# unknownue/puflow

Measured on AMD Instinct MI355X. Metric: patches/sec x4 2048->8192 (PU1K discrete, eval), higher is better.
Workload: dtype f32 (split-fp16 MFMA products, fp32 accumulate); 1 GPU; BASELINE configs[1]: PU1K discrete x4 inference, 32 x 2048-pt patches per GPU (fp32-parity mode); patches_per_gpu=32, total_batch=32, npoint=2048

## Files before the change

include/puflow_hip.h:

```cpp
#ifndef PUFLOW_HIP_H
#define PUFLOW_HIP_H

#ifdef __cplusplus
extern "C" {
#endif

#define PF_OK 0
#define PF_ERR_NULL (-1)
#define PF_ERR_SHAPE (-2)
#define PF_ERR_UNSUPPORTED (-3)
#define PF_ERR_LAUNCH (-4)
#define PF_ERR_WORKSPACE (-5)

int pf_version(void);
const char* pf_error_string(int code);

int pf_knn(const float* p1, const float* p2, int B, int N, int M, int K, int* idx_out, float* dist_out, void* stream);

int pf_nn1(const float* p1, const float* p2, int B, int N, int M, float* dist_out, int* idx_out, void* stream);

int pf_edgeconv(int cfg, const float* pq_or_xyz, const float* tab, const int* idx, const float* wfrag, float* out,
                int B, int N, void* stream);

int pf_edgeconv_tuned(int cfg, int variant, const float* pq_or_xyz, const float* tab, const int* idx,
                      const float* wfrag, float* out, int B, int N, void* stream);

int pf_edgeconv_pq(int unit, const float* pq_or_xyz, const int* idx, const float* wfrag, float* out, const float* w,
                   const long long* off, float* pq_next, int B, int N, int fuse, void* stream);

int pf_pq_gemm(int unit, const float* h, const float* w, const long long* off, float* pq_next, int T, void* stream);
int pf_cond(int unit, const float* h, const float* w, const long long* off, float* c, float* st, float* cp, int T,
            void* stream);
int pf_post(int unit, const float* h, const float* w, const long long* off, float* c, float* st, float* cp,
            float* pq_next, int T, void* stream);
int pf_test_act_pairn(const float* x, int n, float inv, float slope, unsigned* old_h, unsigned* old_l, unsigned* new_h,
                      unsigned* new_l, void* stream);
int pf_cond_all(const float* const* h, const float* w, const long long* off, float* const* c, float* st, float* cp, int T,
                void* stream);

int pf_flow_fwd(const float* xyz, const float* cp, const float* st, const float* w, float* z, float* ld_pt, int T,
                void* stream);

int pf_flow_inv(const float* u, const float* cp, const float* st, const float* w, float* x, int T, int R, void* stream);

int pf_logp(const float* z, const float* ld_pt, float ld_const, int B, int N, float* ldj, float* lpsum, float* logp,
            void* stream);

long long pf_flow_fwd_logp_ws_floats(int B, int N);
int pf_flow_fwd_logp(const float* xyz, const float* cp, const float* st, const float* w, float* z, float* ld_pt,
                     float ld_const, int B, int N, float* ldj, float* lpsum, float* logp, float* ws, void* stream);

int pf_interp(const float* xyz, const float* z, const int* idx16, const float* w, const long long* off, float* u_out,
              int B, int N, int R, void* stream);

int pf_interp_weights(const float* xyz, const int* idx16, const float* w, const long long* off, float* aw_out, int B, int N,
                      void* stream);
int pf_flow_inv_interp(const float* aw, const float* z, const int* idx16, const float* cp, const float* st, const float* w,
                       float* x, int B, int N, int R, void* stream);

int pf_chamfer_fwd(const float* x, const float* y, int B, int N, int M, float* dist1, int* idx1, float* dist2,
                   int* idx2, float* per_sample, float* mean_sum, void* stream);

int pf_chamfer_bwd(const float* x, const float* y, const int* idx1, const int* idx2, const float* g1, const float* g2,
                   float* gx, float* gy, int B, int N, int M, void* stream);
int pf_chamfer_bwd_det(const float* x, const float* y, const int* idx1, const int* idx2, const float* g1, const float* g2,
                       float* gx, float* gy, int B, int N, int M, void* stream);

int pf_emd_forward(const float* xyz1, const float* xyz2, float* dist, int* assignment, float* price,
                   int* assignment_inv, int* bid, float* bid_increments, float* max_increments, int* unass_idx,
                   int* max_idx, float eps, int iters, int B, int n, void* stream);

int pf_emd_forward_ex(const float* xyz1, const float* xyz2, float* dist, int* assignment, float* price,
                      int* assignment_inv, int* bid, float* bid_increments, float* max_increments, int* unass_idx,
// ... 410 lines not shown
```

puflow_amd/csrc/flow.hip:

```cpp
#include <hip/hip_runtime.h>
#include "pf_api_internal.h"
#include "pf_mfma.h"
#include "pf_wave.h"

#ifndef PF_FLOW_NW
#define PF_FLOW_NW 16
#endif
#ifndef PF_FLOW_NW_FWD
#define PF_FLOW_NW_FWD 16
#endif

namespace {

constexpr int FLOW_REC = 5360;
constexpr float LOG2PI_F = 1.8378770664093453f;

struct FlowArgs {
    const float* in;
    const float* cp;
    const float* st;
    const float* w;
    float* out;
    float* ld_pt;
    int T;
    int R;
    int rows;
    int ntiles;
    float* part;
    unsigned* counter;
    float* ldj; float* lps; float* logp;
    float ld_const;
    int B, N;
    const float* aw;
    const float* z;
    const int* idx;
};

struct FlowCond { f4 cp[4]; f4 s0, s1; };

__device__ __forceinline__ FlowCond flow_cond(const float* __restrict__ cp, const float* __restrict__ st, int T, int u,
                                              int pt, int q) {
    FlowCond c;
    const float* cr = cp + ((size_t)u * T + pt) * 64 + 4 * q;
#pragma unroll
    for (int cb = 0; cb < 4; ++cb) c.cp[cb] = *reinterpret_cast<const f4*>(cr + cb * 16);
    const float* sr = st + ((size_t)u * T + pt) * 8;
    c.s0 = *reinterpret_cast<const f4*>(sr);
    c.s1 = *reinterpret_cast<const f4*>(sr + 4);
    return c;
}

template <int TD>
__device__ __forceinline__ void coupling_net(const float* rec , int lane, int q, const FlowCond& c,
                                             const float (&h1)[2], float (&o)[2]) {
    PfPairN hp[1][2];
    const float i2 = rec[5352], i4 = rec[5353];
    {
        f4 hid[4];
#pragma unroll
        for (int cb = 0; cb < 4; ++cb) {
            const f4 wa = *reinterpret_cast<const f4*>(rec + 5200 + (cb * 16 + 4 * q) * 2);
            const f4 wb = *reinterpret_cast<const f4*>(rec + 5200 + (cb * 16 + 4 * q) * 2 + 4);
            f4 v = c.cp[cb];
            v.x = fmaf(wa.x, h1[0], v.x); v.y = fmaf(wa.z, h1[0], v.y);
            v.z = fmaf(wb.x, h1[0], v.z); v.w = fmaf(wb.z, h1[0], v.w);
// ... 7 lines not shown
        hp[0][1] = pf_act_pairn(hid[2], hid[3], 0.01f);
    }
    const PfW2Lds ws{reinterpret_cast<const u4*>(rec), lane};
    f4 h2[1][4];
#pragma unroll
    for (int ob = 0; ob < 4; ++ob) h2[0][ob] = pf_bias(rec + 5120, ob, q);
    pf_mmn<false, 4, 2, 2>(ws, 0, hp, h2);
    hp[0][0] = pf_act_pairn(h2[0][0], h2[0][1], i2, 0.01f);
    hp[0][1] = pf_act_pairn(h2[0][2], h2[0][3], i2, 0.01f);
    f4 acc[1][1];
    acc[0][0] = *reinterpret_cast<const f4*>(rec + 5184 + 4 * q);
    pf_mmn<false, 1, 2, 2>(ws, 8, hp, acc);
    o[0] = acc[0][0].x * i4; o[1] = acc[0][0].y * i4;
}

template <bool INV, int NW>
__global__ __launch_bounds__(NW * 64) void flow_kernel(FlowArgs a) {
    const int lane = threadIdx.x & 63, wave = threadIdx.x >> 6;
    const int col = lane & 15, q = lane >> 4;
    __shared__ f4 wl[6 * FLOW_REC / 4];
    pf_stage_lds(wl, reinterpret_cast<const f4*>(a.w), 6 * FLOW_REC / 4);
    __syncthreads();
    const float* wlf = reinterpret_cast<const float*>(wl);

    for (int tile = blockIdx.x; tile < a.ntiles; tile += gridDim.x) {
        const int g = (tile * NW + wave) * 16 + col;
        const bool ok = g < a.rows;
        const int row = ok ? g : a.rows - 1;
        const int pt = row / a.R;
        float v[3], ld = 0.f;
        if (INV && a.aw) {
            const int r = row - pt * a.R, bN = (pt / a.N) * a.N;
            const int4 j0 = *reinterpret_cast<const int4*>(a.idx + (size_t)pt * 16), j1 = *reinterpret_cast<const int4*>(a.idx + (size_t)pt * 16 + 4);
            const int jj[8] = {j0.x, j0.y, j0.z, j0.w, j1.x, j1.y, j1.z, j1.w};
            float sk[8][3];
#pragma unroll
            for (int k = 0; k < 8; ++k) {
                const float wk = a.aw[((size_t)pt * 8 + k) * 4 + r];
                const float* zz = a.z + (size_t)(bN + jj[k]) * 3;
#pragma unroll
                for (int c = 0; c < 3; ++c) sk[k][c] = __fmul_rn(wk, zz[c]);
            }
#pragma unroll
            for (int c = 0; c < 3; ++c)
                v[c] = __fadd_rn(__fadd_rn(__fadd_rn(sk[0][c], sk[1][c]), __fadd_rn(sk[2][c], sk[3][c])),
                                 __fadd_rn(__fadd_rn(sk[4][c], sk[5][c]), __fadd_rn(sk[6][c], sk[7][c])));
        } else {
#pragma unroll
            for (int c = 0; c < 3; ++c) v[c] = a.in[(size_t)row * 3 + c];
        }
        FlowCond cn = flow_cond(a.cp, a.st, a.T, INV ? 5 : 0, pt, q);

        pf_static_for<0, 6>([&](auto uc) {
            constexpr int i = decltype(uc)::value;
            constexpr int u = INV ? 5 - i : i;
            constexpr int TD = (u % 2 == 0) ? 1 : 2;
            const float* rec = wlf + u * FLOW_REC;
            const float* fc = rec + 5328;
            const FlowCond c = cn;
            if constexpr (i < 5) cn = flow_cond(a.cp, a.st, a.T, INV ? u - 1 : u + 1, pt, q);
            __builtin_amdgcn_sched_barrier(0);
            const float s[3] = {c.s0.x, c.s0.y, c.s0.z}, t[3] = {c.s0.w, c.s1.x, c.s1.y};
            float h1[2], o[2];
            if constexpr (!INV) {
                const float x0 = v[0], x1 = v[1], x2 = v[2];
#pragma unroll
                for (int k = 0; k < 3; ++k)
                    v[k] = fmaf(fc[3 * k + 2], x2, fmaf(fc[3 * k + 1], x1, fmaf(fc[3 * k], x0, fc[9 + k])));
                h1[0] = v[0]; h1[1] = v[1];
                coupling_net<TD>(rec, lane, q, c, h1, o);
                if (TD == 1) { v[1] -= o[0]; v[2] -= o[1]; } else { v[2] -= o[0]; }
                const float y0 = v[2], y1 = v[1], y2 = v[0];
                v[0] = (y0 - t[0]) * expf(-s[0]);
                v[1] = (y1 - t[1]) * expf(-s[1]);
                v[2] = (y2 - t[2]) * expf(-s[2]);
                ld -= (s[0] + s[1]) + s[2];
            } else {
                const float y0 = fmaf(v[0], expf(s[0]), t[0]);
                const float y1 = fmaf(v[1], expf(s[1]), t[1]);
                const float y2 = fmaf(v[2], expf(s[2]), t[2]);
                v[0] = y2; v[1] = y1; v[2] = y0;
                h1[0] = v[0]; h1[1] = v[1];
                coupling_net<TD>(rec, lane, q, c, h1, o);
                if (TD == 1) { v[1] += o[0]; v[2] += o[1]; } else { v[2] += o[0]; }
                const float x0 = v[0], x1 = v[1], x2 = v[2];
#pragma unroll
                for (int k = 0; k < 3; ++k)
                    v[k] = fmaf(fc[12 + 3 * k + 2], x2, fmaf(fc[12 + 3 * k + 1], x1, fmaf(fc[12 + 3 * k], x0, fc[21 + k])));
            }
        });

        if (ok && q == 0) {
            a.out[(size_t)row * 3 + 0] = v[0];
            a.out[(size_t)row * 3 + 1] = v[1];
            a.out[(size_t)row * 3 + 2] = v[2];
// ... 39 lines not shown
                a.lps[b] = accz + l;
                if (b < NW * 64) sa[b] = accz + l;
            }
        }
        __syncthreads();
        float tot = 0.f;
        if (tid == 0)
            for (int b = 0; b < a.B; ++b) tot += b < NW * 64 ? sa[b] : a.lps[b];
        if (tid == 0) {
            *a.logp = -tot / (float)a.B;
            PF_ST(a.counter, 0u);
        }
    }
}

template <bool INV, int NW>
int launch_nw(FlowArgs a, hipStream_t s) {
    a.ntiles = (a.rows + NW * 16 - 1) / (NW * 16);
    const int grid = a.ntiles < 256 ? a.ntiles : 256;
    hipLaunchKernelGGL((flow_kernel<INV, NW>), dim3(grid), dim3(NW * 64), 0, s, a);
    return pf_last_launch_status();
}

template <bool INV>
int launch(FlowArgs a, hipStream_t s) {
    constexpr int NWMAX = INV ? PF_FLOW_NW : PF_FLOW_NW_FWD;
    const int wt = (a.rows + 15) / 16;
    if (wt >= 200 * NWMAX) return launch_nw<INV, NWMAX>(a, s);
    if (wt >= 200 * 8) return launch_nw<INV, 8>(a, s);
    return launch_nw<INV, 4>(a, s);
}

__global__ __launch_bounds__(256) void logp_batch_kernel(const float* __restrict__ z, const float* __restrict__ ld_pt,
                                                        float ld_const, int N, float* __restrict__ ldj,
                                                        float* __restrict__ lpsum) {
    __shared__ float sa[256], sb[256];
    const int b = blockIdx.x, tid = threadIdx.x;
    float accl = 0.f, accz = 0.f;
    for (int n = tid; n < N; n += 256) {
        accl += ld_pt[(size_t)b * N + n];
        const float* zz = z + ((size_t)b * N + n) * 3;
        accz += -0.5f * (zz[0] * zz[0] + LOG2PI_F) + -0.5f * (zz[1] * zz[1] + LOG2PI_F) + -0.5f * (zz[2] * zz[2] + LOG2PI_F);
    }
    sa[tid] = accl; sb[tid] = accz;
    __syncthreads();
// ... 33 lines not shown
                                float ld_const, int B, int N, float* ldj, float* lpsum, float* logp, float* ws, void* stream) {
    if (!xyz || !cp || !st || !w || !z || !ld_pt || !ldj || !lpsum || !logp || !ws) return PF_ERR_NULL;
    if (B <= 0 || N <= 0 || (long long)B * N > (1ll << 30)) return PF_ERR_SHAPE;
    const int T = B * N;
    if (N % 16 != 0) {
        const int rc = pf_flow_fwd(xyz, cp, st, w, z, ld_pt, T, stream);
        return rc != PF_OK ? rc : pf_logp(z, ld_pt, ld_const, B, N, ldj, lpsum, logp, stream);
    }
    FlowArgs a{};
    a.in = xyz; a.cp = cp; a.st = st; a.w = w; a.out = z; a.ld_pt = ld_pt; a.T = T; a.R = 1; a.rows = T;
    a.part = ws; a.counter = reinterpret_cast<unsigned*>(ws + 2 * (T / 16));
    a.ldj = ldj; a.lps = lpsum; a.logp = logp; a.ld_const = ld_const; a.B = B; a.N = N;
    return launch<false>(a, (hipStream_t)stream);
}

extern "C" int pf_flow_inv(const float* u, const float* cp, const float* st, const float* w, float* x, int T, int R,
                           void* stream) {
    if (!u || !cp || !st || !w || !x) return PF_ERR_NULL;
    if (T <= 0 || R <= 0 || (long long)T * R > (1ll << 30)) return PF_ERR_SHAPE;
    FlowArgs a{};
    a.in = u; a.cp = cp; a.st = st; a.w = w; a.out = x; a.ld_pt = nullptr; a.T = T; a.R = R; a.rows = T * R;
    return launch<true>(a, (hipStream_t)stream);
}

extern "C" int pf_flow_inv_interp(const float* aw, const float* z, const int* idx16, const float* cp, const float* st, const float* w,
                                  float* x, int B, int N, int R, void* stream) {
    if (!aw || !z || !idx16 || !cp || !st || !w || !x) return PF_ERR_NULL;
    if (B <= 0 || N < 8 || (long long)B * N * R > (1ll << 30)) return PF_ERR_SHAPE;
    if (R < 1 || R > 4) return PF_ERR_UNSUPPORTED;
    FlowArgs a{};
    a.in = nullptr; a.cp = cp; a.st = st; a.w = w; a.out = x; a.ld_pt = nullptr; a.T = B * N; a.R = R; a.rows = B * N * R;
    a.aw = aw; a.z = z; a.idx = idx16; a.N = N;
    return launch<true>(a, (hipStream_t)stream);
}

extern "C" int pf_logp(const float* z, const float* ld_pt, float ld_const, int B, int N, float* ldj, float* lpsum,
                       float* logp, void* stream) {
    if (!z || !ld_pt || !ldj || !lpsum || !logp) return PF_ERR_NULL;
    if (B <= 0 || N <= 0) return PF_ERR_SHAPE;
    hipStream_t s = (hipStream_t)stream;
    hipLaunchKernelGGL(logp_batch_kernel, dim3(B), dim3(256), 0, s, z, ld_pt, ld_const, N, ldj, lpsum);
    hipLaunchKernelGGL(logp_final_kernel, dim3(1), dim3(64), 0, s, lpsum, B, logp);
    return pf_last_launch_status();
}
```

puflow_amd/csrc/pointwise.hip:

```cpp
#include <hip/hip_runtime.h>
#include "pf_api_internal.h"
#include "pf_mfma.h"
#include "pf_pq.h"

namespace {

struct PqArgs {
    const float* h;
    const u4* w;
    const float* bias;
    const float* scales;
    float* pq;
    int T, ntiles, NT, nrounds;
    float inv;
};

template <int ODIM, int ROWS, int NW>
__global__ __launch_bounds__(NW * 64) void pq_gemm_kernel(PqArgs a) {
    constexpr int HB = ODIM / 16, CP = (HB + 1) / 2, OBT = ROWS / 16, RB = OBT / NW, NTMAX = 16;
    static_assert(OBT % NW == 0, "rows split evenly over the waves");
    const int lane = threadIdx.x & 63, wave = threadIdx.x >> 6;
    const int col = lane & 15, q = lane >> 4;
    __shared__ u4 bl[NTMAX * PQ_TILE_U4<CP>];
    h8 wh[RB][CP], wl[RB][CP];
// ... 33 lines not shown
    nt = nt < 1 ? 1 : (nt > 16 ? 16 : nt);
    a.NT = nt;
    a.nrounds = (a.ntiles + nt - 1) / nt;
    const int grid = a.nrounds < 256 ? a.nrounds : 256;
    hipLaunchKernelGGL((pq_gemm_kernel<ODIM, ROWS, NW>), dim3(grid), dim3(NW * 64), 0, s, a);
    return pf_last_launch_status();
}

struct CondArgs {
    const float* h;
    const float* w;
    long long off[13];
    float* c;
    float* st;
    float* cp;
    int T, ntiles;
    int contiguous;
};

__device__ __forceinline__ f4 pf_scale(f4 v, float k) { return v * k; }

template <int ODIM>
constexpr int cond_lds_bytes() { return ((ODIM / 32) * ((ODIM / 16 + 1) / 2) + 12 * ((ODIM / 32 + 1) / 2) + 20) * 2048; }

template <int ODIM, int CDIM, int NW>
__device__ __forceinline__ void cond_body(const CondArgs& a, u4* wl, int tile0, int tstride) {
    constexpr int HB = ODIM / 16, MB = ODIM / 32, CB = CDIM / 16;
    constexpr int HP = (HB + 1) / 2, MP = (MB + 1) / 2;
    constexpr int F_M1 = 0, F_H1 = F_M1 + MB * HP, F_S2 = F_H1 + 12 * MP, F_T2 = F_S2 + 8, F_ST4 = F_T2 + 8, F_END = F_ST4 + 4;
    const int lane = threadIdx.x & 63, wave = threadIdx.x >> 6;
    const int col = lane & 15, q = lane >> 4;
    static_assert(F_END * 2048 == cond_lds_bytes<ODIM>(), "LDS size formula");
    {
        auto stage = [&](int f0, int nf, long long off) {
            const u4* src = reinterpret_cast<const u4*>(a.w + off);
// ... 74 lines not shown
            PfPairN h1p[1][2];
            h1p[0][0] = pf_act_pairn(h1[0][0], h1[0][1], iH1, 0.01f);
            h1p[0][1] = pf_act_pairn(h1[0][2], h1[0][3], iH1, 0.01f);
            f4 h2[1][4];
#pragma unroll
            for (int o = 0; o < 4; ++o) h2[0][o] = pf_bias(net == 0 ? bS2 : bT2, o, q);
            if constexpr (net == 0) pf_mmn<false, 4, 2, 2>(wsS2, 0, h1p, h2); else pf_mmn<false, 4, 2, 2>(wsT2, 0, h1p, h2);
            const float i2 = net == 0 ? iS2 : iT2;
            h2p[0][2 * net + 0] = pf_act_pairn(h2[0][0], h2[0][1], i2, 0.01f);
            h2p[0][2 * net + 1] = pf_act_pairn(h2[0][2], h2[0][3], i2, 0.01f);
        });
        {
            f4 acc[1][1];
            acc[0][0] = pf_bias(bST4, 0, q);
            pf_mmn<false, 1, 4, 4>(wsST4, 0, h2p, acc);
            if (ok && q < 2) *reinterpret_cast<f4*>(a.st + (size_t)pt * 8 + 4 * q) = pf_scale(acc[0][0], iST4);
        }
    }
}

#ifndef PF_COND_NW
#define PF_COND_NW 12
#endif
constexpr int COND_NW = PF_COND_NW;

template <int ODIM, int CDIM>
__global__ __launch_bounds__(COND_NW * 64) void cond_kernel(CondArgs a) {
    extern __shared__ u4 cond_lds[];
    cond_body<ODIM, CDIM, COND_NW>(a, cond_lds, blockIdx.x, gridDim.x);
}

// ... 81 lines not shown
                       int T, void* stream) {
    if (!h || !w || !off || !st || !cp) return PF_ERR_NULL;
    if (T <= 0) return PF_ERR_SHAPE;
    CondArgs a{};
    a.h = h; a.w = w; a.c = c; a.st = st; a.cp = cp; a.T = T;
    for (int i = 0; i < 13; ++i) a.off[i] = off[i];
    hipStream_t s = (hipStream_t)stream;
    switch (unit) {
        case 0: return launch_cond<32, 32>(a, s);
        case 1: return launch_cond<64, 64>(a, s);
        case 2: case 3: case 4: case 5: return launch_cond<128, 128>(a, s);
        default: return PF_ERR_UNSUPPORTED;
    }
}

extern "C" int pf_cond_all(const float* const* h, const float* w, const long long* off, float* const* c, float* st, float* cp,
                           int T, void* stream) {
    if (!h || !w || !off || (!st != !cp) || (!st && !c)) return PF_ERR_NULL;
    if (T <= 0) return PF_ERR_SHAPE;
    CondAllArgs g{};
    const int ntiles = (T + 15) / 16;
    const int wgt = (ntiles + COND_NW - 1) / COND_NW;
    static const int share_big[6] = {32, 32, 48, 48, 48, 48}, share_small[6] = {24, 32, 50, 50, 50, 50};
    const int* share = wgt <= 50 ? share_small : share_big;
    g.first[0] = 0;
    for (int u = 0; u < 6; ++u) {
        if (!h[u]) return PF_ERR_NULL;
        CondArgs& a = g.u[u];
        a.h = h[u]; a.w = w; a.c = c ? c[u] : nullptr; a.st = st ? st + (size_t)u * T * 8 : nullptr; a.cp = cp ? cp + (size_t)u * T * 64 : nullptr; a.T = T;
        a.ntiles = ntiles;
        for (int i = 0; i < 13; ++i) a.off[i] = off[u * 13 + i];
        a.contiguous = cond_contiguous(a.off, u == 0 ? 32 : (u == 1 ? 64 : 128));
        const int n = wgt < share[u] ? wgt : share[u];
        g.first[u + 1] = g.first[u] + n;
    }
    constexpr int lds = cond_lds_bytes<128>();
    allow_lds(cond_all_kernel, lds);
    hipLaunchKernelGGL(cond_all_kernel, dim3(g.first[6]), dim3(COND_NW * 64), lds, (hipStream_t)stream, g);
    return pf_last_launch_status();
}

extern "C" int pf_post(int unit, const float* h, const float* w, const long long* off, float* c, float* st, float* cp,
                       float* pq_next, int T, void* stream) {
    if (unit < 5) {
        if (!pq_next) return PF_ERR_NULL;
        const int rc = pf_pq_gemm(unit, h, w, off, pq_next, T, stream);
        if (rc != PF_OK) return rc;
    }
    return pf_cond(unit, h, w, off, c, st, cp, T, stream);
}

namespace {
__global__ void act_pairn_test_kernel(const float* __restrict__ x, int n8, float inv, float slope, u4* __restrict__ old_h,
                                      u4* __restrict__ old_l, u4* __restrict__ new_h, u4* __restrict__ new_l) {
// ... 5 lines not shown
    old_h[i] = __builtin_bit_cast(u4, o.h); old_l[i] = __builtin_bit_cast(u4, o.l);
    new_h[i] = __builtin_bit_cast(u4, n.h); new_l[i] = __builtin_bit_cast(u4, n.l);
}
}

extern "C" int pf_test_act_pairn(const float* x, int n, float inv, float slope, unsigned* old_h, unsigned* old_l,
                                 unsigned* new_h, unsigned* new_l, void* stream) {
    if (!x || !old_h || !old_l || !new_h || !new_l) return PF_ERR_NULL;
    if (n <= 0 || n % 8 != 0) return PF_ERR_SHAPE;
    const int n8 = n / 8;
    hipLaunchKernelGGL(act_pairn_test_kernel, dim3((n8 + 63) / 64), dim3(64), 0, (hipStream_t)stream, x, n8, inv, slope,
                       reinterpret_cast<u4*>(old_h), reinterpret_cast<u4*>(old_l), reinterpret_cast<u4*>(new_h),
                       reinterpret_cast<u4*>(new_l));
    return pf_last_launch_status();
}
```

puflow_amd/interpflow.py:

```python
from __future__ import annotations

import os
from typing import List, Optional, Tuple

import numpy as np
import torch
import torch.nn as nn
from torch import Tensor

from . import _lib
from .packing import COND_CHANNELS, FEAT_CHANNELS, GROWTH, NUM_BLOCKS, fold_state_dict, pack_plan

_EC_CFG = [0, 1, 2, 2, 2, 2]
_CHECK_FINITE = os.environ.get("PF_CHECK_FINITE", "0") == "1"


def _conv_bn(cin: int, cout: int, slope: float) -> nn.Sequential:
    return nn.Sequential(nn.Conv2d(cin, cout, kernel_size=1), nn.BatchNorm2d(cout), nn.LeakyReLU(slope))


class _EdgeConvParams(nn.Module):

    def __init__(self, cin: int, odim: int, growth: int):
        super().__init__()
# ... 60 lines not shown
    def __init__(self):
        super().__init__()
        self.knn_context = _Holder()
        self.knn_context.distance_encoder = _Holder()
        self.knn_context.distance_encoder.mlp = nn.Sequential(
            *_conv_bn(10, 64, 0.01), *_conv_bn(64, 64, 0.01), nn.Conv2d(64, 128, kernel_size=1))
        self.knn_context.feat_conv = _EdgeConvParams(3, 128, 16)
        self.weight_unit = _Holder()
        self.weight_unit.mlp = nn.Sequential(
            *_conv_bn(256, 128, 0.01), *_conv_bn(128, 64, 0.01), nn.Conv2d(64, 32, kernel_size=1))


class CondList(list):
    cp: Tensor
    st: Tensor


def _host_state_dict(sd):
    out, groups = {}, {}
    for k, v in sd.items():
        v = v.detach()
        if v.is_cuda:
            groups.setdefault(v.dtype, []).append((k, v))
        else:
            out[k] = v
    for dt, items in groups.items():
        flat = torch.cat([v.reshape(-1) for _, v in items]).cpu()
        pos = 0
        for k, v in items:
            out[k] = flat[pos:pos + v.numel()].reshape(v.shape)
# ... 68 lines not shown
                w = self.ec1n_w[u] if u < 2 else self.ec4_w[u]
                _lib.check(self.lib.pf_edgeconv_pq(u, src, idx16.data_ptr(), self._p(w), h.data_ptr(), self.base, self.post[u],
                                                   nxt.data_ptr(), B, N, self.fuse_pq, s), f"pf_edgeconv_pq[{u}]")

            def pq_gemm(u=u, h=h, nxt=nxt):
                _lib.check(self.lib.pf_pq_gemm(u, h.data_ptr(), self.base, self.post[u], nxt.data_ptr(), T, s), f"pf_pq_gemm[{u}]")

            if u + 1 == NUM_BLOCKS:
                yield h, [(f"edgeconv{u}", ec)]
            elif fused:
                yield h, [(f"edgeconv{u}+pq", ec_pq)]
            else:
                yield h, [(f"edgeconv{u}", ec), (f"pq{u}", pq_gemm)]

    def features(self, xyz: Tensor, idx16: Tensor, want_cs: bool, cs_only: bool = False):
        B, N, _ = xyz.shape
        T, dev, s = B * N, xyz.device, self._stream()
        cp = torch.empty((NUM_BLOCKS, T, 64), dtype=torch.float32, device=dev) if not (cs_only and want_cs) else None
        st = torch.empty((NUM_BLOCKS, T, 8), dtype=torch.float32, device=dev) if not (cs_only and want_cs) else None
        hs: List[Tensor] = []
        for h, calls in self._unit_chain(xyz, idx16):
            for _, call in calls:
                call()
            hs.append(h)
        cs: List[Optional[Tensor]] = [torch.empty((B, N, COND_CHANNELS[u]), dtype=torch.float32, device=dev) if want_cs else None
                                      for u in range(NUM_BLOCKS)]
        self._cond_all(hs, cs if want_cs else None, st, cp, T, s)
        return (cs if want_cs else None), cp, st

    def _cond_all(self, hs, cs, st: Optional[Tensor], cp: Optional[Tensor], T: int, s) -> None:
        import ctypes
        PtrArr = ctypes.c_void_p * NUM_BLOCKS
        h_arr = PtrArr(*[h.data_ptr() for h in hs])
        c_arr = PtrArr(*[c.data_ptr() for c in cs]) if cs is not None else None
        _lib.check(self.lib.pf_cond_all(h_arr, self.base, self.post_all, c_arr, st.data_ptr() if st is not None else None,
                                        cp.data_ptr() if cp is not None else None, T, s), "pf_cond_all")

    def logp_ws(self, B: int, N: int, dev) -> Tensor:
        return torch.zeros((int(self.lib.pf_flow_fwd_logp_ws_floats(B, N)),), dtype=torch.float32, device=dev)

    def flow_f(self, xyz: Tensor, cp: Tensor, st: Tensor, ws: Optional[Tensor] = None):
        B, N, _ = xyz.shape
        T, dev, s = B * N, xyz.device, self._stream()
        z = torch.empty((B, N, 3), dtype=torch.float32, device=dev)
        ld_pt = torch.empty((T,), dtype=torch.float32, device=dev)
        ldj = torch.empty((B,), dtype=torch.float32, device=dev)
        lps = torch.empty((B,), dtype=torch.float32, device=dev)
        logp = torch.empty((), dtype=torch.float32, device=dev)
        if ws is None:
            key = (B, N, s)
            ws = self._logp_ws.get(key)
# ... 6 lines not shown

    def interp(self, xyz: Tensor, z: Tensor, idx16: Tensor, R: int) -> Tensor:
        B, N, _ = xyz.shape
        u = torch.empty((B, N * R, 3), dtype=torch.float32, device=xyz.device)
        _lib.check(self.lib.pf_interp(xyz.data_ptr(), z.data_ptr(), idx16.data_ptr(), self.base, self.interp_off,
                                      u.data_ptr(), B, N, R, self._stream()), "pf_interp")
        return u

    def interp_weights(self, xyz: Tensor, idx16: Tensor) -> Tensor:
        B, N, _ = xyz.shape
        aw = torch.empty((B * N, 8, 4), dtype=torch.float32, device=xyz.device)
        _lib.check(self.lib.pf_interp_weights(xyz.data_ptr(), idx16.data_ptr(), self.base, self.interp_off, aw.data_ptr(), B, N,
                                              self._stream()), "pf_interp_weights")
        return aw

    def flow_g_interp(self, aw: Tensor, z: Tensor, idx16: Tensor, cp: Tensor, st: Tensor, R: int) -> Tensor:
        B, N, _ = z.shape
        x = torch.empty((B, N * R, 3), dtype=torch.float32, device=z.device)
        _lib.check(self.lib.pf_flow_inv_interp(aw.data_ptr(), z.data_ptr(), idx16.data_ptr(), cp.data_ptr(), st.data_ptr(),
                                               self._p(self.flow), x.data_ptr(), B, N, R, self._stream()), "pf_flow_inv_interp")
        return x

    def side_stream(self) -> "torch.cuda.Stream":
        if self._side is None:
            self._side = torch.cuda.Stream(device=self.device)
        return self._side

    def split_interp_for(self, T: int, R: int) -> bool:
        return R <= 4 and self.split_interp == 1

    def flow_g(self, u: Tensor, cp: Tensor, st: Tensor, R: int) -> Tensor:
        B, NR, _ = u.shape
        T = B * NR // R
        x = torch.empty_like(u)
        _lib.check(self.lib.pf_flow_inv(u.data_ptr(), cp.data_ptr(), st.data_ptr(), self._p(self.flow), x.data_ptr(),
                                        T, R, self._stream()), "pf_flow_inv")
        return x


    def profile_stages(self, xyz: Tensor, iters: int = 5, R: int = 4) -> dict:
        B, N, _ = xyz.shape
        T, dev, s = B * N, xyz.device, self._stream()
        acc: dict = {}

        def timed(name, fn):
            a, b = torch.cuda.Event(enable_timing=True), torch.cuda.Event(enable_timing=True)
            a.record()
            r = fn()
            b.record()
            acc.setdefault(name, []).append((a, b))
            return r

        for _ in range(iters + 1):
            idx16 = timed("knn", lambda: self.knn(xyz))
            cp = torch.empty((NUM_BLOCKS, T, 64), dtype=torch.float32, device=dev)
            st = torch.empty((NUM_BLOCKS, T, 8), dtype=torch.float32, device=dev)
            hs = []
            for h, calls in self._unit_chain(xyz, idx16, split_two_launch=True):
                for name, call in calls:
                    timed(name, call)
                hs.append(h)
            timed("cond_all", lambda: self._cond_all(hs, None, st, cp, T, s))
            z, _, _ = timed("flow_f+logp", lambda: self.flow_f(xyz, cp, st))
            u_ = timed("interp", lambda: self.interp(xyz, z, idx16, R))
            timed("flow_g", lambda: self.flow_g(u_, cp, st, R))
        torch.cuda.synchronize()
        return {k: sum(a.elapsed_time(b) for a, b in v[1:]) / (len(v) - 1) for k, v in acc.items()}


class PointInterpFlow(nn.Module):

    def __init__(self, pc_channel: int = 3):
        super().__init__()
        if pc_channel != 3:
            raise ValueError("the HIP path is built for 3-D points (pc_channel=3)")
        self.num_blocks = NUM_BLOCKS
        self.num_neighbors = 16
        self.interp = _InterpParams()
        self.feat_convs = nn.ModuleList(
            [_EdgeConvParams(FEAT_CHANNELS[i], FEAT_CHANNELS[i + 1], GROWTH[i]) for i in range(NUM_BLOCKS)])
# ... 52 lines not shown
    @staticmethod
    def _prep(xyz: Tensor) -> Tensor:
        if not xyz.is_cuda:
            raise _lib.PuflowHipError("input must be a GPU tensor (no CPU fallback)")
        return xyz.detach().contiguous().float()

    def set_to_initialized_state(self) -> None:
        for b in self.flow_blocks:
            b.actnorm.is_inited = True

    @torch.no_grad()
    def feat_extract(self, xyz: Tensor, knn_idx: Tensor) -> CondList:
        self._check_mode()
        xyz = self._prep(xyz)
        e = self._engine(4)
        cs, cp, st = e.features(xyz, knn_idx.to(torch.int32).contiguous(), want_cs=True)
        out = CondList(cs)
        out.cp, out.st = cp, st
        return out

    @torch.no_grad()
    def f(self, xyz: Tensor, cs: CondList) -> Tuple[Tensor, Tensor]:
        self._check_mode()
        z, ldj, _ = self._engine(4).flow_f(self._prep(xyz), cs.cp, cs.st)
        return z, ldj

    @torch.no_grad()
    def log_prob(self, xyz: Tensor, cs: CondList) -> Tuple[Tensor, Tensor]:
        self._check_mode()
        z, _, logp = self._engine(4).flow_f(self._prep(xyz), cs.cp, cs.st)
        return z, logp

    @torch.no_grad()
    def g(self, z: Tensor, cs: CondList, upratio: int) -> Tensor:
        self._check_mode()
        u = torch.flatten(self._prep(z).transpose(2, 3), 1, 2).contiguous()
        return self._engine(upratio).flow_g(u, cs.cp, cs.st, upratio)

    def forward(self, xyz: Tensor, upratio: int = 4) -> Tuple[Tensor, Tensor]:
        if self.training:
            from .train_ops import forward_train
            if not xyz.is_cuda:
                raise _lib.PuflowHipError("input must be a GPU tensor (no CPU fallback)")
            self._train_forwards = getattr(self, "_train_forwards", 0) + 1
            return forward_train(self, xyz, upratio)
        with torch.no_grad():
            return self._forward_eval(xyz, upratio)

    def _forward_eval(self, xyz: Tensor, upratio: int, ws: Optional[Tensor] = None) -> Tuple[Tensor, Tensor]:
        self._check_mode()
        xyz = self._prep(xyz)
        e = self._engine(upratio)
        idx16 = e.knn(xyz)
        if e.split_interp_for(xyz.shape[0] * xyz.shape[1], upratio):
            main, side = torch.cuda.current_stream(), e.side_stream()
            side.wait_stream(main)
            with torch.cuda.stream(side):
                aw = e.interp_weights(xyz, idx16)
            _, cp, st = e.features(xyz, idx16, want_cs=False)
            z, _, logp = e.flow_f(xyz, cp, st, ws)
            main.wait_stream(side)
            aw.record_stream(main)
            x = e.flow_g_interp(aw, z, idx16, cp, st, upratio)
        else:
            _, cp, st = e.features(xyz, idx16, want_cs=False)
            z, _, logp = e.flow_f(xyz, cp, st, ws)
            u = e.interp(xyz, z, idx16, upratio)
            x = e.flow_g(u, cp, st, upratio)
        if _CHECK_FINITE and not bool(torch.isfinite(x).all() & torch.isfinite(logp)):
            raise _lib.PuflowHipError("non-finite output: an activation left the fp16 range of the split-fp16 kernels "
                                      "(or the input holds NaN/inf); check the input normalisation (patch.py:168-178)")
        return x, logp

    @torch.no_grad()
    def forward_stages(self, xyz: Tensor, upratio: int = 4) -> dict:
        self._check_mode()
        xyz = self._prep(xyz)
        e = self._engine(upratio)
        idx16 = e.knn(xyz)
        cs, cp, st = e.features(xyz, idx16, want_cs=True)
        z, ldj, logp = e.flow_f(xyz, cp, st)
        u = e.interp(xyz, z, idx16, upratio)
        x = e.flow_g(u, cp, st, upratio)
        B, N, _ = xyz.shape
        fz = u.view(B, N, upratio, 3).transpose(2, 3)
        return dict(idx16=idx16, cs=cs, cp=cp, st=st, z=z, ldj=ldj, logp=logp, fz=fz, x=x)

    def sample(self, sparse: Tensor, upratio: int = 4) -> Tensor:
        dense, _ = self(sparse, upratio)
        return dense

    @torch.no_grad()
    def graphed(self, B: int, N: int, upratio: int = 4):
        self._check_mode()
        dev = self.flow_blocks[0].actnorm.logs.device
        static_in = torch.zeros((B, N, 3), dtype=torch.float32, device=dev)
        side = torch.cuda.Stream(device=dev)
        side.wait_stream(torch.cuda.current_stream(dev))
        with torch.cuda.stream(side):
            self._forward_eval(static_in, upratio)
            ws = self._engine(upratio).logp_ws(B, N, dev)
# ... 27 lines not shown
```

Baseline: 28900 patches/s.

## Precompute exp(s) per point in cond kernel and reuse in inverse flow

The conditioning kernel now writes exp(s) for each point and flow block into a new es buffer, using lane permutes to gather the three s values. The inverse flow reads es instead of calling expf once per upsampled row, so the R-fold repeated exponentials move into a single per-point pass. The inverse flow also switches to buffer-resource loads with 32-bit offsets when T is small enough, keeping the wide pointer path for large T. This costs an extra buffer that must be written and read back, plus inline permlane asm.

```diff
diff --git a/include/puflow_hip.h b/include/puflow_hip.h
--- a/include/puflow_hip.h
+++ b/include/puflow_hip.h
@@ -37,11 +37,16 @@
                       unsigned* new_l, void* stream);
 int pf_cond_all(const float* const* h, const float* w, const long long* off, float* const* c, float* st, float* cp, int T,
                 void* stream);
+int pf_cond_all_es(const float* const* h, const float* w, const long long* off, float* const* c, float* st, float* cp,
+                   float* es, int T, void* stream);
+int pf_test_expf(const float* x, int n, float* y, void* stream);
 
 int pf_flow_fwd(const float* xyz, const float* cp, const float* st, const float* w, float* z, float* ld_pt, int T,
                 void* stream);
 
 int pf_flow_inv(const float* u, const float* cp, const float* st, const float* w, float* x, int T, int R, void* stream);
+int pf_flow_inv_es(const float* u, const float* cp, const float* st, const float* es, const float* w, float* x, int T, int R,
+                   void* stream);
 
 int pf_logp(const float* z, const float* ld_pt, float ld_const, int B, int N, float* ldj, float* lpsum, float* logp,
             void* stream);
@@ -57,6 +62,8 @@
                       void* stream);
 int pf_flow_inv_interp(const float* aw, const float* z, const int* idx16, const float* cp, const float* st, const float* w,
                        float* x, int B, int N, int R, void* stream);
+int pf_flow_inv_interp_es(const float* aw, const float* z, const int* idx16, const float* cp, const float* st, const float* es,
+                          const float* w, float* x, int B, int N, int R, void* stream);
 
 int pf_chamfer_fwd(const float* x, const float* y, int B, int N, int M, float* dist1, int* idx1, float* dist2,
                    int* idx2, float* per_sample, float* mean_sum, void* stream);
diff --git a/puflow_amd/csrc/flow.hip b/puflow_amd/csrc/flow.hip
--- a/puflow_amd/csrc/flow.hip
+++ b/puflow_amd/csrc/flow.hip
@@ -19,6 +19,7 @@
     const float* in;
     const float* cp;
     const float* st;
+    const float* es;
     const float* w;
     float* out;
     float* ld_pt;
@@ -36,19 +37,54 @@
     const int* idx;
 };
 
-struct FlowCond { f4 cp[4]; f4 s0, s1; };
-
-__device__ __forceinline__ FlowCond flow_cond(const float* __restrict__ cp, const float* __restrict__ st, int T, int u,
-                                              int pt, int q) {
-    FlowCond c;
-    const float* cr = cp + ((size_t)u * T + pt) * 64 + 4 * q;
-#pragma unroll
-    for (int cb = 0; cb < 4; ++cb) c.cp[cb] = *reinterpret_cast<const f4*>(cr + cb * 16);
-    const float* sr = st + ((size_t)u * T + pt) * 8;
-    c.s0 = *reinterpret_cast<const f4*>(sr);
-    c.s1 = *reinterpret_cast<const f4*>(sr + 4);
-    return c;
-}
+struct FlowCond { f4 cp[4]; f4 s0, s1; f4 es; };
+
+template <bool WIDE>
+struct FlowSrc;
+
+template <>
+struct FlowSrc<false> {
+    __amdgpu_buffer_rsrc_t rcp, rst, res;
+    int T, ocp, ost, oes;
+    __device__ __forceinline__ FlowSrc(const float* cp, const float* st, const float* es, int T_)
+        : rcp(__builtin_amdgcn_make_buffer_rsrc(const_cast<float*>(cp), 0, 0x7fffffff, 0x00020000)),
+          rst(__builtin_amdgcn_make_buffer_rsrc(const_cast<float*>(st), 0, 0x7fffffff, 0x00020000)),
+          res(__builtin_amdgcn_make_buffer_rsrc(const_cast<float*>(es), 0, 0x7fffffff, 0x00020000)), T(T_) {}
+    __device__ __forceinline__ void tile(int pt, int q) { ocp = pt * 256 + 16 * q; ost = pt * 32; oes = pt * 16; }
+    template <bool ES>
+    __device__ __forceinline__ FlowCond load(int u) const {
+        FlowCond c;
+#pragma unroll
+        for (int cb = 0; cb < 4; ++cb)
+            c.cp[cb] = __builtin_bit_cast(f4, __builtin_amdgcn_raw_buffer_load_b128(rcp, ocp + cb * 64, u * T * 256, 0));
+        c.s0 = __builtin_bit_cast(f4, __builtin_amdgcn_raw_buffer_load_b128(rst, ost, u * T * 32, 0));
+        c.s1 = __builtin_bit_cast(f4, __builtin_amdgcn_raw_buffer_load_b128(rst, ost + 16, u * T * 32, 0));
+        if constexpr (ES) c.es = __builtin_bit_cast(f4, __builtin_amdgcn_raw_buffer_load_b128(res, oes, u * T * 16, 0));
+        return c;
+    }
+};
+
+template <>
+struct FlowSrc<true> {
+    const float *cp, *st, *es;
+    int T, pt, q;
+    __device__ __forceinline__ FlowSrc(const float* cp_, const float* st_, const float* es_, int T_) : cp(cp_), st(st_), es(es_), T(T_) {}
+    __device__ __forceinline__ void tile(int pt_, int q_) { pt = pt_; q = q_; }
+    template <bool ES>
+    __device__ __forceinline__ FlowCond load(int u) const {
+        FlowCond c;
+        const float* cr = cp + ((size_t)u * T + pt) * 64 + 4 * q;
+#pragma unroll
+        for (int cb = 0; cb < 4; ++cb) c.cp[cb] = *reinterpret_cast<const f4*>(cr + cb * 16);
+        const float* sr = st + ((size_t)u * T + pt) * 8;
+        c.s0 = *reinterpret_cast<const f4*>(sr);
+        c.s1 = *reinterpret_cast<const f4*>(sr + 4);
+        if constexpr (ES) c.es = *reinterpret_cast<const f4*>(es + ((size_t)u * T + pt) * 4);
+        return c;
+    }
+};
+
+inline bool flow_narrow(int T) { return 6ll * T * 256 < (1ll << 31); }
 
 template <int TD>
 __device__ __forceinline__ void coupling_net(const float* rec , int lane, int q, const FlowCond& c,
@@ -86,14 +122,16 @@
     o[0] = acc[0][0].x * i4; o[1] = acc[0][0].y * i4;
 }
 
-template <bool INV, int NW>
+template <bool INV, int NW, bool ES = false, bool WIDE = false>
 __global__ __launch_bounds__(NW * 64) void flow_kernel(FlowArgs a) {
+    static_assert(INV || !ES, "flow f evaluates expf(-s) itself");
     const int lane = threadIdx.x & 63, wave = threadIdx.x >> 6;
     const int col = lane & 15, q = lane >> 4;
     __shared__ f4 wl[6 * FLOW_REC / 4];
     pf_stage_lds(wl, reinterpret_cast<const f4*>(a.w), 6 * FLOW_REC / 4);
     __syncthreads();
     const float* wlf = reinterpret_cast<const float*>(wl);
+    FlowSrc<WIDE> src(a.cp, a.st, a.es, a.T);
 
     for (int tile = blockIdx.x; tile < a.ntiles; tile += gridDim.x) {
         const int g = (tile * NW + wave) * 16 + col;
@@ -121,7 +159,8 @@
 #pragma unroll
             for (int c = 0; c < 3; ++c) v[c] = a.in[(size_t)row * 3 + c];
         }
-        FlowCond cn = flow_cond(a.cp, a.st, a.T, INV ? 5 : 0, pt, q);
+        src.tile(pt, q);
+        FlowCond cn = src.template load<ES>(INV ? 5 : 0);
 
         pf_static_for<0, 6>([&](auto uc) {
             constexpr int i = decltype(uc)::value;
@@ -130,7 +169,7 @@
             const float* rec = wlf + u * FLOW_REC;
             const float* fc = rec + 5328;
             const FlowCond c = cn;
-            if constexpr (i < 5) cn = flow_cond(a.cp, a.st, a.T, INV ? u - 1 : u + 1, pt, q);
+            if constexpr (i < 5) cn = src.template load<ES>(INV ? u - 1 : u + 1);
             __builtin_amdgcn_sched_barrier(0);
             const float s[3] = {c.s0.x, c.s0.y, c.s0.z}, t[3] = {c.s0.w, c.s1.x, c.s1.y};
             float h1[2], o[2];
@@ -148,9 +187,10 @@
                 v[2] = (y2 - t[2]) * expf(-s[2]);
                 ld -= (s[0] + s[1]) + s[2];
             } else {
-                const float y0 = fmaf(v[0], expf(s[0]), t[0]);
-                const float y1 = fmaf(v[1], expf(s[1]), t[1]);
-                const float y2 = fmaf(v[2], expf(s[2]), t[2]);
+                const float e0 = ES ? c.es.x : expf(s[0]), e1 = ES ? c.es.y : expf(s[1]), e2 = ES ? c.es.z : expf(s[2]);
+                const float y0 = fmaf(v[0], e0, t[0]);
+                const float y1 = fmaf(v[1], e1, t[1]);
+                const float y2 = fmaf(v[2], e2, t[2]);
                 v[0] = y2; v[1] = y1; v[2] = y0;
                 h1[0] = v[0]; h1[1] = v[1];
                 coupling_net<TD>(rec, lane, q, c, h1, o);
@@ -220,21 +260,23 @@
     }
 }
 
-template <bool INV, int NW>
+template <bool INV, int NW, bool ES, bool WIDE = false>
 int launch_nw(FlowArgs a, hipStream_t s) {
     a.ntiles = (a.rows + NW * 16 - 1) / (NW * 16);
     const int grid = a.ntiles < 256 ? a.ntiles : 256;
-    hipLaunchKernelGGL((flow_kernel<INV, NW>), dim3(grid), dim3(NW * 64), 0, s, a);
+    hipLaunchKernelGGL((flow_kernel<INV, NW, ES, WIDE>), dim3(grid), dim3(NW * 64), 0, s, a);
     return pf_last_launch_status();
 }
 
-template <bool INV>
+template <bool INV, bool ES = false>
 int launch(FlowArgs a, hipStream_t s) {
     constexpr int NWMAX = INV ? PF_FLOW_NW : PF_FLOW_NW_FWD;
     const int wt = (a.rows + 15) / 16;
-    if (wt >= 200 * NWMAX) return launch_nw<INV, NWMAX>(a, s);
-    if (wt >= 200 * 8) return launch_nw<INV, 8>(a, s);
-    return launch_nw<INV, 4>(a, s);
+    static_assert(200ll * NWMAX * 16 * 6 * 256 < (1ll << 31), "a T that needs the wide form takes the NWMAX launch");
+    if (!flow_narrow(a.T)) return launch_nw<INV, NWMAX, ES, true>(a, s);
+    if (wt >= 200 * NWMAX) return launch_nw<INV, NWMAX, ES>(a, s);
+    if (wt >= 200 * 8) return launch_nw<INV, 8, ES>(a, s);
+    return launch_nw<INV, 4, ES>(a, s);
 }
 
 __global__ __launch_bounds__(256) void logp_batch_kernel(const float* __restrict__ z, const float* __restrict__ ld_pt,
@@ -298,24 +340,34 @@
     return launch<false>(a, (hipStream_t)stream);
 }
 
-extern "C" int pf_flow_inv(const float* u, const float* cp, const float* st, const float* w, float* x, int T, int R,
-                           void* stream) {
+extern "C" int pf_flow_inv_es(const float* u, const float* cp, const float* st, const float* es, const float* w, float* x, int T,
+                              int R, void* stream) {
     if (!u || !cp || !st || !w || !x) return PF_ERR_NULL;
     if (T <= 0 || R <= 0 || (long long)T * R > (1ll << 30)) return PF_ERR_SHAPE;
     FlowArgs a{};
-    a.in = u; a.cp = cp; a.st = st; a.w = w; a.out = x; a.ld_pt = nullptr; a.T = T; a.R = R; a.rows = T * R;
-    return launch<true>(a, (hipStream_t)stream);
-}
-
-extern "C" int pf_flow_inv_interp(const float* aw, const float* z, const int* idx16, const float* cp, const float* st, const float* w,
-                                  float* x, int B, int N, int R, void* stream) {
+    a.in = u; a.cp = cp; a.st = st; a.es = es; a.w = w; a.out = x; a.ld_pt = nullptr; a.T = T; a.R = R; a.rows = T * R;
+    return es ? launch<true, true>(a, (hipStream_t)stream) : launch<true>(a, (hipStream_t)stream);
+}
+
+extern "C" int pf_flow_inv(const float* u, const float* cp, const float* st, const float* w, float* x, int T, int R,
+                           void* stream) {
+    return pf_flow_inv_es(u, cp, st, nullptr, w, x, T, R, stream);
+}
+
+extern "C" int pf_flow_inv_interp_es(const float* aw, const float* z, const int* idx16, const float* cp, const float* st,
+                                     const float* es, const float* w, float* x, int B, int N, int R, void* stream) {
     if (!aw || !z || !idx16 || !cp || !st || !w || !x) return PF_ERR_NULL;
     if (B <= 0 || N < 8 || (long long)B * N * R > (1ll << 30)) return PF_ERR_SHAPE;
     if (R < 1 || R > 4) return PF_ERR_UNSUPPORTED;
     FlowArgs a{};
-    a.in = nullptr; a.cp = cp; a.st = st; a.w = w; a.out = x; a.ld_pt = nullptr; a.T = B * N; a.R = R; a.rows = B * N * R;
+    a.in = nullptr; a.cp = cp; a.st = st; a.es = es; a.w = w; a.out = x; a.ld_pt = nullptr; a.T = B * N; a.R = R; a.rows = B * N * R;
     a.aw = aw; a.z = z; a.idx = idx16; a.N = N;
-    return launch<true>(a, (hipStream_t)stream);
+    return es ? launch<true, true>(a, (hipStream_t)stream) : launch<true>(a, (hipStream_t)stream);
+}
+
+extern "C" int pf_flow_inv_interp(const float* aw, const float* z, const int* idx16, const float* cp, const float* st, const float* w,
+                                  float* x, int B, int N, int R, void* stream) {
+    return pf_flow_inv_interp_es(aw, z, idx16, cp, st, nullptr, w, x, B, N, R, stream);
 }
 
 extern "C" int pf_logp(const float* z, const float* ld_pt, float ld_const, int B, int N, float* ldj, float* lpsum,
diff --git a/puflow_amd/csrc/pointwise.hip b/puflow_amd/csrc/pointwise.hip
--- a/puflow_amd/csrc/pointwise.hip
+++ b/puflow_amd/csrc/pointwise.hip
@@ -71,11 +71,21 @@
     float* c;
     float* st;
     float* cp;
+    float* es;
     int T, ntiles;
     int contiguous;
 };
 
 __device__ __forceinline__ f4 pf_scale(f4 v, float k) { return v * k; }
+
+__device__ __forceinline__ float pf_row0_xyz(f4 v) {
+    float x, y, z;
+    asm volatile("v_mov_b32 %0, %3\n\tv_mov_b32 %1, %4\n\tv_mov_b32 %2, %5\n\t"
+                 "s_nop 1\n\tv_permlane16_swap_b32 %0, %1\n\t"
+                 "s_nop 1\n\tv_permlane32_swap_b32 %0, %2"
+                 : "=&v"(x), "=&v"(y), "=&v"(z) : "v"(v.x), "v"(v.y), "v"(v.z));
+    return x;
+}
 
 template <int ODIM>
 constexpr int cond_lds_bytes() { return ((ODIM / 32) * ((ODIM / 16 + 1) / 2) + 12 * ((ODIM / 32 + 1) / 2) + 20) * 2048; }
@@ -180,7 +190,12 @@
             f4 acc[1][1];
             acc[0][0] = pf_bias(bST4, 0, q);
             pf_mmn<false, 1, 4, 4>(wsST4, 0, h2p, acc);
-            if (ok && q < 2) *reinterpret_cast<f4*>(a.st + (size_t)pt * 8 + 4 * q) = pf_scale(acc[0][0], iST4);
+            const f4 sv = pf_scale(acc[0][0], iST4);
+            if (ok && q < 2) *reinterpret_cast<f4*>(a.st + (size_t)pt * 8 + 4 * q) = sv;
+            if (a.es) {
+                const float e = expf(pf_row0_xyz(sv));
+                if (ok) a.es[(size_t)pt * 4 + q] = q < 3 ? e : 0.f;
+            }
         }
     }
 }
@@ -292,9 +307,9 @@
     }
 }
 
-extern "C" int pf_cond_all(const float* const* h, const float* w, const long long* off, float* const* c, float* st, float* cp,
-                           int T, void* stream) {
-    if (!h || !w || !off || (!st != !cp) || (!st && !c)) return PF_ERR_NULL;
+extern "C" int pf_cond_all_es(const float* const* h, const float* w, const long long* off, float* const* c, float* st, float* cp,
+                              float* es, int T, void* stream) {
+    if (!h || !w || !off || (!st != !cp) || (!st && !c) || (es && !st)) return PF_ERR_NULL;
     if (T <= 0) return PF_ERR_SHAPE;
     CondAllArgs g{};
     const int ntiles = (T + 15) / 16;
@@ -306,6 +321,7 @@
         if (!h[u]) return PF_ERR_NULL;
         CondArgs& a = g.u[u];
         a.h = h[u]; a.w = w; a.c = c ? c[u] : nullptr; a.st = st ? st + (size_t)u * T * 8 : nullptr; a.cp = cp ? cp + (size_t)u * T * 64 : nullptr; a.T = T;
+        a.es = es ? es + (size_t)u * T * 4 : nullptr;
         a.ntiles = ntiles;
         for (int i = 0; i < 13; ++i) a.off[i] = off[u * 13 + i];
         a.contiguous = cond_contiguous(a.off, u == 0 ? 32 : (u == 1 ? 64 : 128));
@@ -316,6 +332,11 @@
     allow_lds(cond_all_kernel, lds);
     hipLaunchKernelGGL(cond_all_kernel, dim3(g.first[6]), dim3(COND_NW * 64), lds, (hipStream_t)stream, g);
     return pf_last_launch_status();
+}
+
+extern "C" int pf_cond_all(const float* const* h, const float* w, const long long* off, float* const* c, float* st, float* cp,
+                           int T, void* stream) {
+    return pf_cond_all_es(h, w, off, c, st, cp, nullptr, T, stream);
 }
 
 extern "C" int pf_post(int unit, const float* h, const float* w, const long long* off, float* c, float* st, float* cp,
@@ -351,3 +372,17 @@
                        reinterpret_cast<u4*>(new_l));
     return pf_last_launch_status();
 }
+
+namespace {
+__global__ void expf_test_kernel(const float* __restrict__ x, int n, float* __restrict__ y) {
+    const int i = blockIdx.x * blockDim.x + threadIdx.x;
+    if (i < n) y[i] = expf(x[i]);
+}
+}
+
+extern "C" int pf_test_expf(const float* x, int n, float* y, void* stream) {
+    if (!x || !y) return PF_ERR_NULL;
+    if (n <= 0) return PF_ERR_SHAPE;
+    hipLaunchKernelGGL(expf_test_kernel, dim3((n + 255) / 256), dim3(256), 0, (hipStream_t)stream, x, n, y);
+    return pf_last_launch_status();
+}
diff --git a/puflow_amd/interpflow.py b/puflow_amd/interpflow.py
--- a/puflow_amd/interpflow.py
+++ b/puflow_amd/interpflow.py
@@ -98,6 +98,7 @@
 class CondList(list):
     cp: Tensor
     st: Tensor
+    es: Tensor
 
 
 def _host_state_dict(sd):
@@ -196,10 +197,14 @@
                 yield h, [(f"edgeconv{u}", ec), (f"pq{u}", pq_gemm)]
 
     def features(self, xyz: Tensor, idx16: Tensor, want_cs: bool, cs_only: bool = False):
+        return self.features_es(xyz, idx16, want_cs, cs_only, want_es=False)[:3]
+
+    def features_es(self, xyz: Tensor, idx16: Tensor, want_cs: bool, cs_only: bool = False, want_es: bool = True):
         B, N, _ = xyz.shape
         T, dev, s = B * N, xyz.device, self._stream()
         cp = torch.empty((NUM_BLOCKS, T, 64), dtype=torch.float32, device=dev) if not (cs_only and want_cs) else None
         st = torch.empty((NUM_BLOCKS, T, 8), dtype=torch.float32, device=dev) if not (cs_only and want_cs) else None
+        es = torch.empty((NUM_BLOCKS, T, 4), dtype=torch.float32, device=dev) if want_es and st is not None else None
         hs: List[Tensor] = []
         for h, calls in self._unit_chain(xyz, idx16):
             for _, call in calls:
@@ -207,16 +212,17 @@
             hs.append(h)
         cs: List[Optional[Tensor]] = [torch.empty((B, N, COND_CHANNELS[u]), dtype=torch.float32, device=dev) if want_cs else None
                                       for u in range(NUM_BLOCKS)]
-        self._cond_all(hs, cs if want_cs else None, st, cp, T, s)
-        return (cs if want_cs else None), cp, st
-
-    def _cond_all(self, hs, cs, st: Optional[Tensor], cp: Optional[Tensor], T: int, s) -> None:
+        self._cond_all(hs, cs if want_cs else None, st, cp, T, s, es)
+        return (cs if want_cs else None), cp, st, es
+
+    def _cond_all(self, hs, cs, st: Optional[Tensor], cp: Optional[Tensor], T: int, s, es: Optional[Tensor] = None) -> None:
         import ctypes
         PtrArr = ctypes.c_void_p * NUM_BLOCKS
         h_arr = PtrArr(*[h.data_ptr() for h in hs])
         c_arr = PtrArr(*[c.data_ptr() for c in cs]) if cs is not None else None
-        _lib.check(self.lib.pf_cond_all(h_arr, self.base, self.post_all, c_arr, st.data_ptr() if st is not None else None,
-                                        cp.data_ptr() if cp is not None else None, T, s), "pf_cond_all")
+        _lib.check(self.lib.pf_cond_all_es(h_arr, self.base, self.post_all, c_arr, st.data_ptr() if st is not None else None,
+                                           cp.data_ptr() if cp is not None else None,
+                                           es.data_ptr() if es is not None else None, T, s), "pf_cond_all_es")
 
     def logp_ws(self, B: int, N: int, dev) -> Tensor:
         return torch.zeros((int(self.lib.pf_flow_fwd_logp_ws_floats(B, N)),), dtype=torch.float32, device=dev)
@@ -253,11 +259,13 @@
                                               self._stream()), "pf_interp_weights")
         return aw
 
-    def flow_g_interp(self, aw: Tensor, z: Tensor, idx16: Tensor, cp: Tensor, st: Tensor, R: int) -> Tensor:
+    def flow_g_interp(self, aw: Tensor, z: Tensor, idx16: Tensor, cp: Tensor, st: Tensor, R: int,
+                      es: Optional[Tensor] = None) -> Tensor:
         B, N, _ = z.shape
         x = torch.empty((B, N * R, 3), dtype=torch.float32, device=z.device)
-        _lib.check(self.lib.pf_flow_inv_interp(aw.data_ptr(), z.data_ptr(), idx16.data_ptr(), cp.data_ptr(), st.data_ptr(),
-                                               self._p(self.flow), x.data_ptr(), B, N, R, self._stream()), "pf_flow_inv_interp")
+        _lib.check(self.lib.pf_flow_inv_interp_es(aw.data_ptr(), z.data_ptr(), idx16.data_ptr(), cp.data_ptr(), st.data_ptr(),
+                                                  es.data_ptr() if es is not None else None, self._p(self.flow), x.data_ptr(),
+                                                  B, N, R, self._stream()), "pf_flow_inv_interp_es")
         return x
 
     def side_stream(self) -> "torch.cuda.Stream":
@@ -268,12 +276,12 @@
     def split_interp_for(self, T: int, R: int) -> bool:
         return R <= 4 and self.split_interp == 1
 
-    def flow_g(self, u: Tensor, cp: Tensor, st: Tensor, R: int) -> Tensor:
+    def flow_g(self, u: Tensor, cp: Tensor, st: Tensor, R: int, es: Optional[Tensor] = None) -> Tensor:
         B, NR, _ = u.shape
         T = B * NR // R
         x = torch.empty_like(u)
-        _lib.check(self.lib.pf_flow_inv(u.data_ptr(), cp.data_ptr(), st.data_ptr(), self._p(self.flow), x.data_ptr(),
-                                        T, R, self._stream()), "pf_flow_inv")
+        _lib.check(self.lib.pf_flow_inv_es(u.data_ptr(), cp.data_ptr(), st.data_ptr(), es.data_ptr() if es is not None else None,
+                                           self._p(self.flow), x.data_ptr(), T, R, self._stream()), "pf_flow_inv_es")
         return x
 
 
@@ -294,15 +302,16 @@
             idx16 = timed("knn", lambda: self.knn(xyz))
             cp = torch.empty((NUM_BLOCKS, T, 64), dtype=torch.float32, device=dev)
             st = torch.empty((NUM_BLOCKS, T, 8), dtype=torch.float32, device=dev)
+            es = torch.empty((NUM_BLOCKS, T, 4), dtype=torch.float32, device=dev)
             hs = []
             for h, calls in self._unit_chain(xyz, idx16, split_two_launch=True):
                 for name, call in calls:
                     timed(name, call)
                 hs.append(h)
-            timed("cond_all", lambda: self._cond_all(hs, None, st, cp, T, s))
+            timed("cond_all", lambda: self._cond_all(hs, None, st, cp, T, s, es))
             z, _, _ = timed("flow_f+logp", lambda: self.flow_f(xyz, cp, st))
             u_ = timed("interp", lambda: self.interp(xyz, z, idx16, R))
-            timed("flow_g", lambda: self.flow_g(u_, cp, st, R))
+            timed("flow_g", lambda: self.flow_g(u_, cp, st, R, es))
         torch.cuda.synchronize()
         return {k: sum(a.elapsed_time(b) for a, b in v[1:]) / (len(v) - 1) for k, v in acc.items()}
 
@@ -385,9 +394,9 @@
         self._check_mode()
         xyz = self._prep(xyz)
         e = self._engine(4)
-        cs, cp, st = e.features(xyz, knn_idx.to(torch.int32).contiguous(), want_cs=True)
+        cs, cp, st, es = e.features_es(xyz, knn_idx.to(torch.int32).contiguous(), want_cs=True)
         out = CondList(cs)
-        out.cp, out.st = cp, st
+        out.cp, out.st, out.es = cp, st, es
         return out
 
     @torch.no_grad()
@@ -406,7 +415,7 @@
     def g(self, z: Tensor, cs: CondList, upratio: int) -> Tensor:
         self._check_mode()
         u = torch.flatten(self._prep(z).transpose(2, 3), 1, 2).contiguous()
-        return self._engine(upratio).flow_g(u, cs.cp, cs.st, upratio)
+        return self._engine(upratio).flow_g(u, cs.cp, cs.st, upratio, getattr(cs, "es", None))
 
     def forward(self, xyz: Tensor, upratio: int = 4) -> Tuple[Tensor, Tensor]:
         if self.training:
@@ -428,16 +437,16 @@
             side.wait_stream(main)
             with torch.cuda.stream(side):
                 aw = e.interp_weights(xyz, idx16)
-            _, cp, st = e.features(xyz, idx16, want_cs=False)
+            _, cp, st, es = e.features_es(xyz, idx16, want_cs=False)
             z, _, logp = e.flow_f(xyz, cp, st, ws)
             main.wait_stream(side)
             aw.record_stream(main)
-            x = e.flow_g_interp(aw, z, idx16, cp, st, upratio)
+            x = e.flow_g_interp(aw, z, idx16, cp, st, upratio, es)
         else:
-            _, cp, st = e.features(xyz, idx16, want_cs=False)
+            _, cp, st, es = e.features_es(xyz, idx16, want_cs=False)
             z, _, logp = e.flow_f(xyz, cp, st, ws)
             u = e.interp(xyz, z, idx16, upratio)
-            x = e.flow_g(u, cp, st, upratio)
+            x = e.flow_g(u, cp, st, upratio, es)
         if _CHECK_FINITE and not bool(torch.isfinite(x).all() & torch.isfinite(logp)):
             raise _lib.PuflowHipError("non-finite output: an activation left the fp16 range of the split-fp16 kernels "
                                       "(or the input holds NaN/inf); check the input normalisation (patch.py:168-178)")
@@ -449,13 +458,13 @@
         xyz = self._prep(xyz)
         e = self._engine(upratio)
         idx16 = e.knn(xyz)
-        cs, cp, st = e.features(xyz, idx16, want_cs=True)
+        cs, cp, st, es = e.features_es(xyz, idx16, want_cs=True)
         z, ldj, logp = e.flow_f(xyz, cp, st)
         u = e.interp(xyz, z, idx16, upratio)
-        x = e.flow_g(u, cp, st, upratio)
+        x = e.flow_g(u, cp, st, upratio, es)
         B, N, _ = xyz.shape
         fz = u.view(B, N, upratio, 3).transpose(2, 3)
-        return dict(idx16=idx16, cs=cs, cp=cp, st=st, z=z, ldj=ldj, logp=logp, fz=fz, x=x)
+        return dict(idx16=idx16, cs=cs, cp=cp, st=st, es=es, z=z, ldj=ldj, logp=logp, fz=fz, x=x)
 
     def sample(self, sparse: Tensor, upratio: int = 4) -> Tensor:
         dense, _ = self(sparse, upratio)
```

After: 28900 patches/s. Within noise of the previous version (-0.0%).
